# YuejiangDong/MAL

Measured on AMD Instinct MI355X. Metric: train images/sec at B=12 192x640 KITTI-shaped (MAL loss path: passes A+B+C fwd+bwd), higher is better.
Workload: dtype f32

## Files before the change

### mal_amd/csrc/mal_dyn.hip

```cpp
#include "mal_common.h"
#include "mal_device.h"

namespace mal {

MAL_DEV size_t dyn_row(const long long* sel, int i, int rows) {
  long long r = sel ? sel[i] : (long long)i;
  if (rows > 0) r = r < 0 ? 0 : (r >= rows ? (long long)rows - 1 : r);
  return (size_t)r;
}

struct DynParams {
  const uint8_t* mask_last; const uint8_t* mask_next;
  const long long* idx_last; const long long* idx_next;
  int rows_last, rows_next;
  int num, C, H, W, replace;
  const float* img_last; const float* img_next;
  float* ori_last; float* ori_next;
  int* ext;
  int* delta;
  uint8_t* flags;
  const float* g_ori_last; const float* g_ori_next; float* g_img_last; float* g_img_next;
  int prefilled;
  float* g_tmp_last; float* g_tmp_next;
};

constexpr int kDynBatch = 16;
struct DynBatch { DynParams s[kDynBatch]; };
constexpr int kExtChunks = 8;

__global__ __launch_bounds__(1024) void dyn_extents_kernel(DynBatch bt) {
  extern __shared__ int sh[];
  const DynParams& p = bt.s[blockIdx.z];
  if ((int)blockIdx.x >= p.num) return;
  const int i = blockIdx.x, which = blockIdx.y / kExtChunks, chunk = blockIdx.y % kExtChunks, tid = threadIdx.x;
  const int H = p.H, W = p.W;
  const int band = (H + kExtChunks - 1) / kExtChunks, r_lo = chunk * band, r_hi = min(r_lo + band, H);
  const int k_lo = r_lo * W, HW = max(r_hi, r_lo) * W;
  int* rowf = sh;
  int* colf = sh + H;
  int* res = sh + H + W;
  for (int k = tid; k < H + W; k += 1024) sh[k] = 0;
  if (tid < 4) res[tid] = (tid & 1) ? 0x7fffffff : 0;
  __syncthreads();
  const long long* sel = which ? p.idx_next : p.idx_last;
  const uint8_t* m = (which ? p.mask_next : p.mask_last) + dyn_row(sel, i, which ? p.rows_next : p.rows_last) * ((size_t)H * W);
  auto mark = [&](int k) { rowf[k / W] = 1; colf[k % W] = 1; };
  if ((HW & 15) == 0 && (k_lo & 15) == 0 && (reinterpret_cast<size_t>(m) & 15) == 0) {
    const uint4* m16 = reinterpret_cast<const uint4*>(m);
    for (int k = k_lo / 16 + tid; k < HW / 16; k += 1024) {
      const uint4 v = m16[k];
      const unsigned w4[4] = {v.x, v.y, v.z, v.w};
#pragma unroll
      for (int j = 0; j < 4; ++j)
        if (w4[j])
          for (int t = 0; t < 4; ++t)
            if ((w4[j] >> (8 * t)) & 0xffu) mark(k * 16 + j * 4 + t);
    }
  } else {
    for (int k = k_lo + tid; k < HW; k += 1024)
      if (m[k]) mark(k);
  }
  __syncthreads();
  for (int r = 1 + tid; r < H; r += 1024)
    if (rowf[r]) { atomicMax(&res[0], r); atomicMin(&res[1], r); }
  for (int c = 1 + tid; c < W; c += 1024)
    if (colf[c]) { atomicMax(&res[2], c); atomicMin(&res[3], c); }
  __syncthreads();
  if (tid < 4) p.ext[((i * 2 + which) * kExtChunks + chunk) * 4 + tid] = res[tid];
}

MAL_DEV unsigned nz4(unsigned w) {
  return ((w & 0xffu) ? 1u : 0u) | ((w & 0xff00u) ? 2u : 0u) | ((w & 0xff0000u) ? 4u : 0u) | ((w & 0xff000000u) ? 8u : 0u);
}

__global__ __launch_bounds__(1024) void dyn_extents16_kernel(DynBatch bt) {
  __shared__ int res[4];
  const DynParams& p = bt.s[blockIdx.z];
  if ((int)blockIdx.x >= p.num) return;
  const int i = blockIdx.x, which = blockIdx.y / kExtChunks, chunk = blockIdx.y % kExtChunks, tid = threadIdx.x;
  const int H = p.H, W = p.W, W16 = W >> 4;
  const int band = (H + kExtChunks - 1) / kExtChunks, r_lo = chunk * band, r_hi = min(r_lo + band, H);
  if (tid < 4) res[tid] = (tid & 1) ? 0x7fffffff : 0;
  __syncthreads();
  const long long* sel = which ? p.idx_next : p.idx_last;
  const uint4* m16 = reinterpret_cast<const uint4*>((which ? p.mask_next : p.mask_last) +
                                                    dyn_row(sel, i, which ? p.rows_next : p.rows_last) * ((size_t)H * W));
  int rmax = 0, rmin = 0x7fffffff, cmax = 0, cmin = 0x7fffffff;
  for (int k = r_lo * W16 + tid; k < max(r_hi, r_lo) * W16; k += (int)blockDim.x) {
    const uint4 v = m16[k];
    const unsigned w4[4] = {v.x, v.y, v.z, v.w};
    unsigned m = 0u;
#pragma unroll
    for (int j = 0; j < 4; ++j) m |= nz4(w4[j]) << (4 * j);
    if (m) {
      const int row = k / W16, col0 = (k - row * W16) * 16;
      if (row >= 1) { rmax = max(rmax, row); rmin = min(rmin, row); }
      const unsigned m1 = col0 == 0 ? (m & ~1u) : m;
      if (m1) { cmax = max(cmax, col0 + 31 - __clz((int)m1)); cmin = min(cmin, col0 + __ffs((int)m1) - 1); }
    }
  }
  for (int o = 32; o > 0; o >>= 1) {
    rmax = max(rmax, __shfl_down(rmax, o, 64)); rmin = min(rmin, __shfl_down(rmin, o, 64));
    cmax = max(cmax, __shfl_down(cmax, o, 64)); cmin = min(cmin, __shfl_down(cmin, o, 64));
  }
  if ((tid & 63) == 0) {
    if (rmax > 0) { atomicMax(&res[0], rmax); atomicMin(&res[1], rmin); }
    if (cmax > 0) { atomicMax(&res[2], cmax); atomicMin(&res[3], cmin); }
  }
  __syncthreads();
  if (tid < 4) p.ext[((i * 2 + which) * kExtChunks + chunk) * 4 + tid] = res[tid];
}

MAL_DEV void instance_delta(const DynParams& p, int i, int* dx_out, int* dy_out) {
  int el[4], en[4];
#pragma unroll 1
  for (int which = 0; which < 2; ++which) {
    int* e = which ? en : el;
    for (int t = 0; t < 4; ++t) e[t] = (t & 1) ? 0x7fffffff : 0;
    for (int c = 0; c < kExtChunks; ++c)
      for (int t = 0; t < 4; ++t) {
        const int v = p.ext[((i * 2 + which) * kExtChunks + c) * 4 + t];
        e[t] = (t & 1) ? min(e[t], v) : max(e[t], v);
      }
    for (int t = 0; t < 4; ++t)
      if (e[t] == 0x7fffffff) e[t] = 0;
  }
  auto pick = [](int a, int b) {
    const int s = abs(b) > abs(a) ? b : a;
    return (int)rintf((float)s * 0.5f);
  };
  int dx = pick(en[0] - el[0], en[1] - el[1]);
  int dy = pick(en[2] - el[2], en[3] - el[3]);
  if (p.replace) { if (abs(dx) < 3) dx = 0; if (abs(dy) < 3) dy = 0; }
  *dx_out = dx; *dy_out = dy;
}

MAL_DEV void stage_instances(const DynParams& p, int* s_delta, bool from_ext) {
  if (from_ext) {
    for (int i = threadIdx.x; i < p.num; i += 256) {
      int dx, dy;
      instance_delta(p, i, &dx, &dy);
      s_delta[2 * i] = dx; s_delta[2 * i + 1] = dy;
      if (blockIdx.x == 0) { p.delta[2 * i] = dx; p.delta[2 * i + 1] = dy; }
    }
  }
  for (int k = threadIdx.x; k < p.num * 2; k += 256) {
    if (!from_ext) s_delta[k] = p.delta[k];
    const int i = k >> 1;
    const long long* sel = (k & 1) ? p.idx_next : p.idx_last;
    s_delta[2 * p.num + k] = (int)dyn_row(sel, i, (k & 1) ? p.rows_next : p.rows_last);
  }
  __syncthreads();
}

__global__ __launch_bounds__(256) void dyn_synth_fwd_kernel(DynBatch bt) {
  extern __shared__ int s_delta[];
  const DynParams& p = bt.s[blockIdx.z];
  stage_instances(p, s_delta, true);
  const int* s_row = s_delta + 2 * p.num;
  const int H = p.H, W = p.W, HW = H * W;
  const int pix = blockIdx.x * 256 + threadIdx.x;
  if (pix >= HW) return;
  const int r = pix / W, c = pix - r * W;
  bool region = false, any_l = false, any_n = false, bg_l = false, bg_n = false;
  float accl[4] = {0.f, 0.f, 0.f, 0.f}, accn[4] = {0.f, 0.f, 0.f, 0.f};
  for (int i = 0; i < p.num; ++i) {
    const uint8_t* ml = p.mask_last + (size_t)s_row[2 * i] * HW;
    const uint8_t* mn = p.mask_next + (size_t)s_row[2 * i + 1] * HW;
    const bool a = ml[pix] != 0, b = mn[pix] != 0;
    region |= a | b; bg_l |= a & !b; bg_n |= b & !a;
    const int dx = s_delta[2 * i], dy = s_delta[2 * i + 1];
    {
      const int rs = r - dx, cs = c - dy;
      if (rs >= 0 && rs < H && cs >= 0 && cs < W && ml[rs * W + cs]) {
        any_l = true;
        for (int ch = 0; ch < p.C; ++ch) accl[ch] += p.img_last[(size_t)ch * HW + rs * W + cs];
      }
    }
    {
      const int rs = r + dx, cs = c + dy;
      if (rs >= 0 && rs < H && cs >= 0 && cs < W && mn[rs * W + cs]) {
        any_n = true;
        for (int ch = 0; ch < p.C; ++ch) accn[ch] += p.img_next[(size_t)ch * HW + rs * W + cs];
      }
    }
  }
  p.flags[pix] = (uint8_t)((region ? 1 : 0) | (any_l ? 2 : 0) | (any_n ? 4 : 0) | (bg_l ? 8 : 0) | (bg_n ? 16 : 0));
  if (p.prefilled && !region) return;
  for (int ch = 0; ch < p.C; ++ch) {
    const float il = p.img_last[(size_t)ch * HW + pix], in = p.img_next[(size_t)ch * HW + pix];
    p.ori_last[(size_t)ch * HW + pix] = region ? (any_l ? accl[ch] : (bg_l ? in : il)) : il;
    p.ori_next[(size_t)ch * HW + pix] = region ? (any_n ? accn[ch] : (bg_n ? il : in)) : in;
  }
}

template <bool REGION>
__global__ __launch_bounds__(256) void dyn_synth_bwd_kernel(DynBatch bt) {
  extern __shared__ int s_delta[];
  const DynParams& p = bt.s[blockIdx.z];
  stage_instances(p, s_delta, false);
  const int* s_row = s_delta + 2 * p.num;
  const int H = p.H, W = p.W, HW = H * W;
  const int pix = blockIdx.x * 256 + threadIdx.x;
  if (pix >= HW) return;
  const int r = pix / W, c = pix - r * W;
  const int f = p.flags[pix];
  if (REGION && !(f & 1)) return;
  const bool ol_from_l = !(f & 1) || (!(f & 2) && !(f & 8)), ol_from_n = (f & 1) && !(f & 2) && (f & 8);
  const bool on_from_n = !(f & 1) || (!(f & 4) && !(f & 16)), on_from_l = (f & 1) && !(f & 4) && (f & 16);
  float gl[4] = {0.f, 0.f, 0.f, 0.f}, gn[4] = {0.f, 0.f, 0.f, 0.f};
  for (int ch = 0; ch < p.C; ++ch) {
    const float a = p.g_ori_last[(size_t)ch * HW + pix], b = p.g_ori_next[(size_t)ch * HW + pix];
    if (ol_from_l) gl[ch] += a;
    if (on_from_l) gl[ch] += b;
    if (on_from_n) gn[ch] += b;
    if (ol_from_n) gn[ch] += a;
  }
  for (int i = 0; i < p.num; ++i) {
    const int dx = s_delta[2 * i], dy = s_delta[2 * i + 1];
    if (p.mask_last[(size_t)s_row[2 * i] * HW + pix]) {
      const int rd = r + dx, cd = c + dy;
      if (rd >= 0 && rd < H && cd >= 0 && cd < W && (p.flags[rd * W + cd] & 1))
        for (int ch = 0; ch < p.C; ++ch) gl[ch] += p.g_ori_last[(size_t)ch * HW + rd * W + cd];
    }
    if (p.mask_next[(size_t)s_row[2 * i + 1] * HW + pix]) {
      const int rd = r - dx, cd = c - dy;
      if (rd >= 0 && rd < H && cd >= 0 && cd < W && (p.flags[rd * W + cd] & 1))
        for (int ch = 0; ch < p.C; ++ch) gn[ch] += p.g_ori_next[(size_t)ch * HW + rd * W + cd];
    }
  }
  float* const out_l = REGION ? p.g_tmp_last : p.g_img_last;
  float* const out_n = REGION ? p.g_tmp_next : p.g_img_next;
  for (int ch = 0; ch < p.C; ++ch) {
    if (out_l) out_l[(size_t)ch * HW + pix] = gl[ch];
    if (out_n) out_n[(size_t)ch * HW + pix] = gn[ch];
  }
}

__global__ __launch_bounds__(256) void dyn_apply_region_kernel(DynBatch bt) {
  const DynParams& p = bt.s[blockIdx.z];
  const int HW = p.H * p.W;
  const int pix = blockIdx.x * 256 + threadIdx.x;
  if (pix >= HW || !(p.flags[pix] & 1)) return;
  for (int ch = 0; ch < p.C; ++ch) {
    p.g_img_last[(size_t)ch * HW + pix] = p.g_tmp_last[(size_t)ch * HW + pix];
    p.g_img_next[(size_t)ch * HW + pix] = p.g_tmp_next[(size_t)ch * HW + pix];
  }
}

MAL_DEV unsigned bytes4_at(const uint8_t* row, int cs, int W) {
  const unsigned* rw = reinterpret_cast<const unsigned*>(row);
  const int a0 = cs >> 2, sh = (cs & 3) * 8, wmax = (W >> 2) - 1;
  const unsigned l0 = rw[min(max(a0, 0), wmax)], l1 = rw[min(max(a0 + 1, 0), wmax)];
  const unsigned w0 = (a0 >= 0 && a0 <= wmax) ? l0 : 0u, w1 = (a0 + 1 >= 0 && a0 + 1 <= wmax) ? l1 : 0u;
  return sh ? (w0 >> sh) | (w1 << (32 - sh)) : w0;
}

MAL_DEV float4 ld4(const float* p) { return *reinterpret_cast<const float4*>(p); }
MAL_DEV void st4(float* p, const float (&v)[4]) { *reinterpret_cast<float4*>(p) = make_float4(v[0], v[1], v[2], v[3]); }

template <int C>
MAL_DEV void gather_add(float (&acc)[4][C], const float* __restrict__ img, int HW, unsigned sel, int base) {
  const char* plane[C];
#pragma unroll
  for (int ch = 0; ch < C; ++ch) {
    plane[ch] = reinterpret_cast<const char*>(img + (size_t)ch * HW);
    asm volatile("" : "+s"(plane[ch]));
  }
  float v[4][C];
#pragma unroll
  for (int k = 0; k < 4; ++k) {
    const unsigned off = (unsigned)(((sel >> k) & 1u) ? base + k : 0) * 4u;
#pragma unroll
    for (int ch = 0; ch < C; ++ch) v[k][ch] = *(const __attribute__((address_space(1))) float*)(plane[ch] + off);
  }
#pragma unroll
  for (int k = 0; k < 4; ++k)
#pragma unroll
    for (int ch = 0; ch < C; ++ch) {
      acc[k][ch] += ((sel >> k) & 1u) ? v[k][ch] : 0.f;
      asm volatile("" : "+v"(acc[k][ch]));
    }
}

template <int C>
__global__ __launch_bounds__(256) void dyn_synth_fwd4_kernel(DynBatch bt) {
  extern __shared__ int s_delta[];
  const DynParams& p = bt.s[blockIdx.z];
  stage_instances(p, s_delta, true);
  const int* s_row = s_delta + 2 * p.num;
  const int H = p.H, W = p.W, HW = H * W, W4 = W >> 2;
  const int q = blockIdx.x * 256 + threadIdx.x;
  if (q >= (HW >> 2)) return;
  const int r = q / W4, c = (q - r * W4) * 4, pix = r * W + c;
  const float* __restrict__ il = p.img_last;
  const float* __restrict__ in = p.img_next;
  unsigned region = 0u, any_l = 0u, any_n = 0u, bg_l = 0u, bg_n = 0u;
  float accl[4][C], accn[4][C];
#pragma unroll
  for (int k = 0; k < 4; ++k)
#pragma unroll
    for (int ch = 0; ch < C; ++ch) { accl[k][ch] = 0.f; accn[k][ch] = 0.f; }
  for (int i = 0; i < p.num; ++i) {
    const uint8_t* ml = p.mask_last + (size_t)__builtin_amdgcn_readfirstlane(s_row[2 * i]) * HW;
    const uint8_t* mn = p.mask_next + (size_t)__builtin_amdgcn_readfirstlane(s_row[2 * i + 1]) * HW;
    const int dx = __builtin_amdgcn_readfirstlane(s_delta[2 * i]), dy = __builtin_amdgcn_readfirstlane(s_delta[2 * i + 1]);
    const int rl = r - dx, rn = r + dx;
    const unsigned wa = *reinterpret_cast<const unsigned*>(ml + pix), wb = *reinterpret_cast<const unsigned*>(mn + pix);
    const unsigned sl_raw = bytes4_at(ml + (size_t)min(max(rl, 0), H - 1) * W, c - dy, W);
    const unsigned sn_raw = bytes4_at(mn + (size_t)min(max(rn, 0), H - 1) * W, c + dy, W);
    const unsigned a4 = nz4(wa), b4 = nz4(wb);
    const unsigned sl = (rl >= 0 && rl < H) ? nz4(sl_raw) : 0u, sn = (rn >= 0 && rn < H) ? nz4(sn_raw) : 0u;
    region |= a4 | b4; bg_l |= a4 & ~b4; bg_n |= b4 & ~a4;
    any_l |= sl; any_n |= sn;
    if (__any((sl | sn) != 0u)) {
      const int bl = rl * W + (c - dy), bn = rn * W + (c + dy);
      gather_add<C>(accl, il, HW, sl, bl);
      __builtin_amdgcn_sched_barrier(0);
      gather_add<C>(accn, in, HW, sn, bn);
    }
  }
  unsigned fw = 0u;
#pragma unroll
  for (int k = 0; k < 4; ++k)
    fw |= ((((region >> k) & 1u)) | (((any_l >> k) & 1u) << 1) | (((any_n >> k) & 1u) << 2) | (((bg_l >> k) & 1u) << 3) |
           (((bg_n >> k) & 1u) << 4)) << (8 * k);
  *reinterpret_cast<unsigned*>(p.flags + pix) = fw;
  if (p.prefilled && !__any(region != 0u)) return;
  const bool prefilled = p.prefilled != 0;
#pragma unroll
  for (int ch = 0; ch < C; ++ch) {
    const float4 a = ld4(il + (size_t)ch * HW + pix), b = ld4(in + (size_t)ch * HW + pix);
    const float av[4] = {a.x, a.y, a.z, a.w}, bv[4] = {b.x, b.y, b.z, b.w};
    float ol[4], on[4];
#pragma unroll
    for (int k = 0; k < 4; ++k) {
      const bool rg = (region >> k) & 1u;
      ol[k] = rg ? (((any_l >> k) & 1u) ? accl[k][ch] : (((bg_l >> k) & 1u) ? bv[k] : av[k])) : av[k];
      on[k] = rg ? (((any_n >> k) & 1u) ? accn[k][ch] : (((bg_n >> k) & 1u) ? av[k] : bv[k])) : bv[k];
    }
    float* const dl = p.ori_last + (size_t)ch * HW + pix;
    float* const dn = p.ori_next + (size_t)ch * HW + pix;
    if (!prefilled) { st4(dl, ol); st4(dn, on); continue; }
#pragma unroll
    for (int k = 0; k < 4; ++k)
      if ((region >> k) & 1u) { dl[k] = ol[k]; dn[k] = on[k]; }
  }
}

template <int C, bool REGION>
__global__ __launch_bounds__(256) void dyn_synth_bwd4_kernel(DynBatch bt) {
  extern __shared__ int s_delta[];
  const DynParams& p = bt.s[blockIdx.z];
  stage_instances(p, s_delta, false);
  const int* s_row = s_delta + 2 * p.num;
  const int H = p.H, W = p.W, HW = H * W, W4 = W >> 2;
  const int q = blockIdx.x * 256 + threadIdx.x;
  if (q >= (HW >> 2)) return;
  const int r = q / W4, c = (q - r * W4) * 4, pix = r * W + c;
  const float* __restrict__ go_l = p.g_ori_last;
  const float* __restrict__ go_n = p.g_ori_next;
  const unsigned fw = *reinterpret_cast<const unsigned*>(p.flags + pix);
  float* const out_l = REGION ? p.g_tmp_last : p.g_img_last;
  float* const out_n = REGION ? p.g_tmp_next : p.g_img_next;
  const bool wave_region = __any((fw & 0x01010101u) != 0u);
  if (REGION && !wave_region) return;
  float gl[C][4], gn[C][4];
#pragma unroll
  for (int ch = 0; ch < C; ++ch) {
    const float4 a4 = ld4(go_l + (size_t)ch * HW + pix), b4 = ld4(go_n + (size_t)ch * HW + pix);
    const float a[4] = {a4.x, a4.y, a4.z, a4.w}, b[4] = {b4.x, b4.y, b4.z, b4.w};
#pragma unroll
    for (int k = 0; k < 4; ++k) {
      const int f = (int)((fw >> (8 * k)) & 0xffu);
      const bool ol_from_l = !(f & 1) || (!(f & 2) && !(f & 8)), ol_from_n = (f & 1) && !(f & 2) && (f & 8);
      const bool on_from_n = !(f & 1) || (!(f & 4) && !(f & 16)), on_from_l = (f & 1) && !(f & 4) && (f & 16);
      float l = 0.f, n = 0.f;
      l += ol_from_l ? a[k] : 0.f;
      l += on_from_l ? b[k] : 0.f;
      n += on_from_n ? b[k] : 0.f;
      n += ol_from_n ? a[k] : 0.f;
      gl[ch][k] = l; gn[ch][k] = n;
    }
  }
  if (wave_region) {
    for (int i = 0; i < p.num; ++i) {
      const int dx = s_delta[2 * i], dy = s_delta[2 * i + 1];
      const unsigned ma = nz4(*reinterpret_cast<const unsigned*>(p.mask_last + (size_t)s_row[2 * i] * HW + pix));
      const unsigned mb = nz4(*reinterpret_cast<const unsigned*>(p.mask_next + (size_t)s_row[2 * i + 1] * HW + pix));
      const int rdl = r + dx, rdn = r - dx;
      const unsigned fl = bytes4_at(p.flags + (size_t)min(max(rdl, 0), H - 1) * W, c + dy, W);
      const unsigned fn = bytes4_at(p.flags + (size_t)min(max(rdn, 0), H - 1) * W, c - dy, W);
      unsigned hl = 0u, hn = 0u;
#pragma unroll
      for (int k = 0; k < 4; ++k) {
        hl |= (((fl >> (8 * k)) & 1u) & ((ma >> k) & 1u)) << k;
        hn |= (((fn >> (8 * k)) & 1u) & ((mb >> k) & 1u)) << k;
      }
      if (rdl < 0 || rdl >= H) hl = 0u;
      if (rdn < 0 || rdn >= H) hn = 0u;
      if (__any((hl | hn) != 0u)) {
        const int bl = rdl * W + (c + dy), bn = rdn * W + (c - dy);
        float vl[C][4], vn[C][4];
#pragma unroll
        for (int ch = 0; ch < C; ++ch)
#pragma unroll
          for (int k = 0; k < 4; ++k) {
            vl[ch][k] = go_l[(size_t)ch * HW + (((hl >> k) & 1u) ? bl + k : 0)];
            vn[ch][k] = go_n[(size_t)ch * HW + (((hn >> k) & 1u) ? bn + k : 0)];
          }
#pragma unroll
        for (int ch = 0; ch < C; ++ch)
#pragma unroll
          for (int k = 0; k < 4; ++k) {
            gl[ch][k] += ((hl >> k) & 1u) ? vl[ch][k] : 0.f;
            gn[ch][k] += ((hn >> k) & 1u) ? vn[ch][k] : 0.f;
          }
      }
    }
  }
  if (!REGION) {
#pragma unroll
    for (int ch = 0; ch < C; ++ch) {
      if (out_l) st4(out_l + (size_t)ch * HW + pix, gl[ch]);
      if (out_n) st4(out_n + (size_t)ch * HW + pix, gn[ch]);
    }
    return;
  }
#pragma unroll
  for (int k = 0; k < 4; ++k)
    if ((fw >> (8 * k)) & 1u) {
#pragma unroll
      for (int ch = 0; ch < C; ++ch) { out_l[(size_t)ch * HW + pix + k] = gl[ch][k]; out_n[(size_t)ch * HW + pix + k] = gn[ch][k]; }
    }
}

template <int C>
__global__ __launch_bounds__(256) void dyn_apply_region4_kernel(DynBatch bt) {
  const DynParams& p = bt.s[blockIdx.z];
  const int HW = p.H * p.W;
  const int q = blockIdx.x * 256 + threadIdx.x;
  if (q >= (HW >> 2)) return;
  const int pix = q * 4;
  const unsigned fw = *reinterpret_cast<const unsigned*>(p.flags + pix);
  if (!__any((fw & 0x01010101u) != 0u)) return;
  const float* __restrict__ tl = p.g_tmp_last;
  const float* __restrict__ tn = p.g_tmp_next;
  float4 vl[C], vn[C];
#pragma unroll
  for (int ch = 0; ch < C; ++ch) { vl[ch] = ld4(tl + (size_t)ch * HW + pix); vn[ch] = ld4(tn + (size_t)ch * HW + pix); }
#pragma unroll
  for (int ch = 0; ch < C; ++ch) {
    const float a[4] = {vl[ch].x, vl[ch].y, vl[ch].z, vl[ch].w}, b[4] = {vn[ch].x, vn[ch].y, vn[ch].z, vn[ch].w};
#pragma unroll
    for (int k = 0; k < 4; ++k)
      if ((fw >> (8 * k)) & 1u) { p.g_img_last[(size_t)ch * HW + pix + k] = a[k]; p.g_img_next[(size_t)ch * HW + pix + k] = b[k]; }
  }
}

}
namespace mal { opt_t g_dyn_small_blocks{1}; }

using namespace mal;

static bool aligned_to(const void* ptr, size_t a) { return ptr == nullptr || (reinterpret_cast<uintptr_t>(ptr) & (a - 1)) == 0; }

static int dyn_check(int num, int C, int H, int W) {
  if (num < 1 || num > MAL_MAX_INSTANCES || C < 1 || C > 4) return MAL_EINVAL;
  if (H < 2 || W < 2 || (double)H * W > 2.0e9 / 4) return MAL_ESHAPE;
  return MAL_OK;
}

extern "C" size_t mal_dyn_workspace_bytes(int num) {
  return num > 0 ? align256((size_t)num * 8 * kExtChunks * sizeof(int)) : 0;
}

static int dyn_fwd_chunk(const mal_dyn_item* it, int n, int C, int H, int W, int replace, hipStream_t st) {
  DynBatch bt = {};
  int max_num = 0;
  for (int k = 0; k < n; ++k) {
    const mal_dyn_item& a = it[k];
    int rc = dyn_check(a.num, C, H, W);
    if (rc) return rc;
    if (!a.mask_last || !a.mask_next || !a.img_last || !a.img_next || !a.ori_last || !a.ori_next || !a.delta || !a.flags ||
        !a.ws)
      return MAL_EINVAL;
    if (a.ws_bytes < mal_dyn_workspace_bytes(a.num)) return MAL_EWORKSPACE;
    DynParams& p = bt.s[k];
    p.mask_last = a.mask_last; p.mask_next = a.mask_next; p.num = a.num; p.C = C; p.H = H; p.W = W; p.replace = replace;
    p.idx_last = (const long long*)a.idx_last; p.idx_next = (const long long*)a.idx_next;
    p.rows_last = a.n_last; p.rows_next = a.n_next;
    p.img_last = a.img_last; p.img_next = a.img_next; p.ori_last = a.ori_last; p.ori_next = a.ori_next;
    p.ext = (int*)a.ws; p.delta = a.delta; p.flags = a.flags; p.prefilled = a.prefilled;
    max_num = a.num > max_num ? a.num : max_num;
  }
  bool wide = (W & 15) == 0;
  for (int k = 0; k < n && wide; ++k) wide = aligned_to(bt.s[k].mask_last, 16) && aligned_to(bt.s[k].mask_next, 16);
  if (wide)
    hipLaunchKernelGGL(dyn_extents16_kernel, dim3(max_num, 2 * kExtChunks, n), dim3(g_dyn_small_blocks ? 256 : 1024), 0, st, bt);
  else
    hipLaunchKernelGGL(dyn_extents_kernel, dim3(max_num, 2 * kExtChunks, n), dim3(1024), (size_t)(H + W + 4) * sizeof(int), st, bt);
  bool quad = (W & 3) == 0 && C == 3;
  for (int k = 0; k < n && quad; ++k) {
    const DynParams& q = bt.s[k];
    quad = aligned_to(q.mask_last, 4) && aligned_to(q.mask_next, 4) && aligned_to(q.flags, 4) && aligned_to(q.img_last, 16) &&
           aligned_to(q.img_next, 16) && aligned_to(q.ori_last, 16) && aligned_to(q.ori_next, 16);
  }
  if (quad)
    hipLaunchKernelGGL(dyn_synth_fwd4_kernel<3>, dim3((H * W / 4 + 255) / 256, 1, n), dim3(256), (size_t)max_num * 4 * sizeof(int), st, bt);
  else
    hipLaunchKernelGGL(dyn_synth_fwd_kernel, dim3((H * W + 255) / 256, 1, n), dim3(256), (size_t)max_num * 4 * sizeof(int), st, bt);
  return launch_status();
}

static int dyn_bwd_chunk(const mal_dyn_item* it, int n, int C, int H, int W, hipStream_t st) {
  DynBatch bt = {};
  int max_num = 0;
  int region = 0;
  for (int k = 0; k < n; ++k) {
    const mal_dyn_item& a = it[k];
    int rc = dyn_check(a.num, C, H, W);
    if (rc) return rc;
    if (!a.mask_last || !a.mask_next || !a.delta || !a.flags || !a.g_ori_last || !a.g_ori_next ||
        (!a.g_img_last && !a.g_img_next))
      return MAL_EINVAL;
    DynParams& p = bt.s[k];
    p.mask_last = a.mask_last; p.mask_next = a.mask_next; p.num = a.num; p.C = C; p.H = H; p.W = W;
    p.idx_last = (const long long*)a.idx_last; p.idx_next = (const long long*)a.idx_next;
    p.rows_last = a.n_last; p.rows_next = a.n_next;
    p.delta = a.delta; p.flags = a.flags;
    p.g_ori_last = a.g_ori_last; p.g_ori_next = a.g_ori_next; p.g_img_last = a.g_img_last; p.g_img_next = a.g_img_next;
    p.g_tmp_last = a.g_tmp_last; p.g_tmp_next = a.g_tmp_next;
    const bool inplace = a.g_img_last == a.g_ori_last || a.g_img_next == a.g_ori_next;
    if (inplace && (a.g_img_last != a.g_ori_last || a.g_img_next != a.g_ori_next || !a.g_tmp_last || !a.g_tmp_next)) return MAL_EINVAL;
    if (a.region_only) {
      if (inplace || !a.g_img_last || !a.g_img_next) return MAL_EINVAL;
      p.g_tmp_last = a.g_img_last; p.g_tmp_next = a.g_img_next;
    }
    const int form = a.region_only ? 2 : (inplace ? 1 : 0);
    if (k == 0) region = form;
    else if (region != form) return MAL_EINVAL;
    max_num = a.num > max_num ? a.num : max_num;
  }
  bool quad = (W & 3) == 0 && C == 3;
  for (int k = 0; k < n && quad; ++k) {
    const DynParams& q = bt.s[k];
    quad = aligned_to(q.mask_last, 4) && aligned_to(q.mask_next, 4) && aligned_to(q.flags, 4) && aligned_to(q.g_ori_last, 16) && aligned_to(q.g_ori_next, 16) && aligned_to(q.g_img_last, 16) &&
           aligned_to(q.g_img_next, 16) && aligned_to(q.g_tmp_last, 16) && aligned_to(q.g_tmp_next, 16);
  }
  const size_t lds = (size_t)max_num * 4 * sizeof(int);
  const dim3 grid((H * W + 255) / 256, 1, n), grid4((H * W / 4 + 255) / 256, 1, n);
  if (region && quad) {
    hipLaunchKernelGGL((dyn_synth_bwd4_kernel<3, true>), grid4, dim3(256), lds, st, bt);
    if (region == 1) hipLaunchKernelGGL(dyn_apply_region4_kernel<3>, grid4, dim3(256), 0, st, bt);
  } else if (region) {
    hipLaunchKernelGGL(dyn_synth_bwd_kernel<true>, grid, dim3(256), lds, st, bt);
    if (region == 1) hipLaunchKernelGGL(dyn_apply_region_kernel, grid, dim3(256), 0, st, bt);
  } else if (quad) {
    hipLaunchKernelGGL((dyn_synth_bwd4_kernel<3, false>), grid4, dim3(256), lds, st, bt);
  } else {
    hipLaunchKernelGGL(dyn_synth_bwd_kernel<false>, grid, dim3(256), lds, st, bt);
  }
  return launch_status();
}

extern "C" int mal_dyn_batch_fwd(const mal_dyn_item* items, int n_items, int C, int H, int W, int replace, void* stream) {
  if (!items || n_items < 1) return MAL_EINVAL;
  for (int o = 0; o < n_items; o += kDynBatch) {
    int rc = dyn_fwd_chunk(items + o, n_items - o < kDynBatch ? n_items - o : kDynBatch, C, H, W, replace, (hipStream_t)stream);
    if (rc) return rc;
  }
  return MAL_OK;
}

extern "C" int mal_dyn_batch_bwd(const mal_dyn_item* items, int n_items, int C, int H, int W, void* stream) {
  if (!items || n_items < 1) return MAL_EINVAL;
  for (int o = 0; o < n_items; o += kDynBatch) {
    int rc = dyn_bwd_chunk(items + o, n_items - o < kDynBatch ? n_items - o : kDynBatch, C, H, W, (hipStream_t)stream);
    if (rc) return rc;
  }
  return MAL_OK;
}

extern "C" int mal_dyn_instance_fwd(const uint8_t* mask_last, const uint8_t* mask_next, int num, const float* img_last,
                                    const float* img_next, int C, int H, int W, int replace, float* ori_last,
                                    float* ori_next, int32_t* delta, uint8_t* flags, void* ws, size_t ws_bytes,
                                    void* stream) {
  mal_dyn_item a = {};
  a.mask_last = mask_last; a.mask_next = mask_next; a.num = num; a.img_last = img_last; a.img_next = img_next;
  a.ori_last = ori_last; a.ori_next = ori_next; a.delta = delta; a.flags = flags; a.ws = ws; a.ws_bytes = ws_bytes;
  return dyn_fwd_chunk(&a, 1, C, H, W, replace, (hipStream_t)stream);
}

extern "C" int mal_dyn_instance_bwd(const uint8_t* mask_last, const uint8_t* mask_next, int num, const int32_t* delta,
                                    const uint8_t* flags, const float* g_ori_last, const float* g_ori_next, int C, int H,
                                    int W, float* g_img_last, float* g_img_next, void* stream) {
  mal_dyn_item a = {};
  a.mask_last = mask_last; a.mask_next = mask_next; a.num = num; a.delta = const_cast<int32_t*>(delta);
  a.flags = const_cast<uint8_t*>(flags); a.g_ori_last = g_ori_last; a.g_ori_next = g_ori_next;
  a.g_img_last = g_img_last; a.g_img_next = g_img_next;
  return dyn_bwd_chunk(&a, 1, C, H, W, (hipStream_t)stream);
}
```

Measured before the change: 42480.

## Batch instance mask loads in groups and prefetch cotangents in dynamic synth kernels

The forward and backward 4-pixel synth kernels now process instances in groups of three. All mask and flag word loads for a group are issued together before any use, and the backward kernel prefetches the next group and issues cotangent loads before shared-memory staging. Instance staging is reorganised so one thread per (instance, frame) reduces the extents and exchanges them via a shuffle, using a packed int4 record per instance. The extents scan also unrolls four uint4 loads per iteration. These changes aim to hide global-load latency and cut serial per-instance overhead, at the cost of more registers and a forced waves-per-EU setting that could limit occupancy or cause spills.

```diff
diff --git a/mal_amd/csrc/mal_dyn.hip b/mal_amd/csrc/mal_dyn.hip
--- a/mal_amd/csrc/mal_dyn.hip
+++ b/mal_amd/csrc/mal_dyn.hip
@@ -23,6 +23,15 @@
   int prefilled;
   float* g_tmp_last; float* g_tmp_next;
 };
+
+MAL_DEV int dyn_row_of_frame(const DynParams& p, int i, int which) {
+  long long rl = i, rn = i;
+  if (p.idx_last) rl = p.idx_last[i];
+  if (p.idx_next) rn = p.idx_next[i];
+  if (p.rows_last > 0) rl = rl < 0 ? 0 : (rl >= p.rows_last ? (long long)p.rows_last - 1 : rl);
+  if (p.rows_next > 0) rn = rn < 0 ? 0 : (rn >= p.rows_next ? (long long)p.rows_next - 1 : rn);
+  return (int)(which ? rn : rl);
+}
 
 constexpr int kDynBatch = 16;
 struct DynBatch { DynParams s[kDynBatch]; };
@@ -86,8 +95,7 @@
   const uint4* m16 = reinterpret_cast<const uint4*>((which ? p.mask_next : p.mask_last) +
                                                     dyn_row(sel, i, which ? p.rows_next : p.rows_last) * ((size_t)H * W));
   int rmax = 0, rmin = 0x7fffffff, cmax = 0, cmin = 0x7fffffff;
-  for (int k = r_lo * W16 + tid; k < max(r_hi, r_lo) * W16; k += (int)blockDim.x) {
-    const uint4 v = m16[k];
+  auto fold = [&](int k, const uint4& v) {
     const unsigned w4[4] = {v.x, v.y, v.z, v.w};
     unsigned m = 0u;
 #pragma unroll
@@ -98,6 +106,15 @@
       const unsigned m1 = col0 == 0 ? (m & ~1u) : m;
       if (m1) { cmax = max(cmax, col0 + 31 - __clz((int)m1)); cmin = min(cmin, col0 + __ffs((int)m1) - 1); }
     }
+  };
+  const int k_end = max(r_hi, r_lo) * W16, step = (int)blockDim.x;
+  for (int k = r_lo * W16 + tid; k < k_end; k += 4 * step) {
+    int kk[4];
+    uint4 v[4];
+#pragma unroll
+    for (int j = 0; j < 4; ++j) { kk[j] = min(k + j * step, k_end - 1); v[j] = m16[kk[j]]; }
+#pragma unroll
+    for (int j = 0; j < 4; ++j) fold(kk[j], v[j]);
   }
   for (int o = 32; o > 0; o >>= 1) {
     rmax = max(rmax, __shfl_down(rmax, o, 64)); rmin = min(rmin, __shfl_down(rmin, o, 64));
@@ -111,44 +128,49 @@
   if (tid < 4) p.ext[((i * 2 + which) * kExtChunks + chunk) * 4 + tid] = res[tid];
 }
 
-MAL_DEV void instance_delta(const DynParams& p, int i, int* dx_out, int* dy_out) {
-  int el[4], en[4];
-#pragma unroll 1
-  for (int which = 0; which < 2; ++which) {
-    int* e = which ? en : el;
-    for (int t = 0; t < 4; ++t) e[t] = (t & 1) ? 0x7fffffff : 0;
+static_assert(2 * MAL_MAX_INSTANCES <= 256, "stage_extents: one thread per (instance, frame) of a 256-thread workgroup");
+MAL_DEV void stage_extents(const DynParams& p, int* s_delta) {
+  const int t = threadIdx.x;
+  if (t < 2 * p.num) {
+    const int i = t >> 1, which = t & 1;
+    const int* rec = p.ext + (size_t)t * (kExtChunks * 4);
+    int v[kExtChunks][4];
+#pragma unroll
     for (int c = 0; c < kExtChunks; ++c)
-      for (int t = 0; t < 4; ++t) {
-        const int v = p.ext[((i * 2 + which) * kExtChunks + c) * 4 + t];
-        e[t] = (t & 1) ? min(e[t], v) : max(e[t], v);
-      }
-    for (int t = 0; t < 4; ++t)
-      if (e[t] == 0x7fffffff) e[t] = 0;
-  }
-  auto pick = [](int a, int b) {
-    const int s = abs(b) > abs(a) ? b : a;
-    return (int)rintf((float)s * 0.5f);
-  };
-  int dx = pick(en[0] - el[0], en[1] - el[1]);
-  int dy = pick(en[2] - el[2], en[3] - el[3]);
-  if (p.replace) { if (abs(dx) < 3) dx = 0; if (abs(dy) < 3) dy = 0; }
-  *dx_out = dx; *dy_out = dy;
-}
-
-MAL_DEV void stage_instances(const DynParams& p, int* s_delta, bool from_ext) {
-  if (from_ext) {
-    for (int i = threadIdx.x; i < p.num; i += 256) {
-      int dx, dy;
-      instance_delta(p, i, &dx, &dy);
-      s_delta[2 * i] = dx; s_delta[2 * i + 1] = dy;
+#pragma unroll
+      for (int k = 0; k < 4; ++k) v[c][k] = rec[c * 4 + k];
+    const int row = dyn_row_of_frame(p, i, which);
+    int e[4], o[4];
+#pragma unroll
+    for (int k = 0; k < 4; ++k) {
+      e[k] = (k & 1) ? 0x7fffffff : 0;
+#pragma unroll
+      for (int c = 0; c < kExtChunks; ++c) e[k] = (k & 1) ? min(e[k], v[c][k]) : max(e[k], v[c][k]);
+      if (e[k] == 0x7fffffff) e[k] = 0;
+      o[k] = __shfl_xor(e[k], 1, 64);
+    }
+    s_delta[4 * i + 2 + which] = row;
+    if (!which) {
+      auto pick = [](int a, int b) {
+        const int s = abs(b) > abs(a) ? b : a;
+        return (int)rintf((float)s * 0.5f);
+      };
+      int dx = pick(o[0] - e[0], o[1] - e[1]);
+      int dy = pick(o[2] - e[2], o[3] - e[3]);
+      if (p.replace) { if (abs(dx) < 3) dx = 0; if (abs(dy) < 3) dy = 0; }
+      s_delta[4 * i] = dx; s_delta[4 * i + 1] = dy;
       if (blockIdx.x == 0) { p.delta[2 * i] = dx; p.delta[2 * i + 1] = dy; }
     }
   }
-  for (int k = threadIdx.x; k < p.num * 2; k += 256) {
-    if (!from_ext) s_delta[k] = p.delta[k];
-    const int i = k >> 1;
-    const long long* sel = (k & 1) ? p.idx_next : p.idx_last;
-    s_delta[2 * p.num + k] = (int)dyn_row(sel, i, (k & 1) ? p.rows_next : p.rows_last);
+  __syncthreads();
+}
+
+MAL_DEV void stage_instances(const DynParams& p, int* s_delta) {
+  const int k = threadIdx.x;
+  if (k < 2 * p.num) {
+    const int i = k >> 1, d = p.delta[k], row = dyn_row_of_frame(p, i, k & 1);
+    s_delta[4 * i + (k & 1)] = d;
+    s_delta[4 * i + 2 + (k & 1)] = row;
   }
   __syncthreads();
 }
@@ -156,8 +178,7 @@
 __global__ __launch_bounds__(256) void dyn_synth_fwd_kernel(DynBatch bt) {
   extern __shared__ int s_delta[];
   const DynParams& p = bt.s[blockIdx.z];
-  stage_instances(p, s_delta, true);
-  const int* s_row = s_delta + 2 * p.num;
+  stage_extents(p, s_delta);
   const int H = p.H, W = p.W, HW = H * W;
   const int pix = blockIdx.x * 256 + threadIdx.x;
   if (pix >= HW) return;
@@ -165,11 +186,11 @@
   bool region = false, any_l = false, any_n = false, bg_l = false, bg_n = false;
   float accl[4] = {0.f, 0.f, 0.f, 0.f}, accn[4] = {0.f, 0.f, 0.f, 0.f};
   for (int i = 0; i < p.num; ++i) {
-    const uint8_t* ml = p.mask_last + (size_t)s_row[2 * i] * HW;
-    const uint8_t* mn = p.mask_next + (size_t)s_row[2 * i + 1] * HW;
+    const uint8_t* ml = p.mask_last + (size_t)s_delta[4 * i + 2] * HW;
+    const uint8_t* mn = p.mask_next + (size_t)s_delta[4 * i + 3] * HW;
     const bool a = ml[pix] != 0, b = mn[pix] != 0;
     region |= a | b; bg_l |= a & !b; bg_n |= b & !a;
-    const int dx = s_delta[2 * i], dy = s_delta[2 * i + 1];
+    const int dx = s_delta[4 * i], dy = s_delta[4 * i + 1];
     {
       const int rs = r - dx, cs = c - dy;
       if (rs >= 0 && rs < H && cs >= 0 && cs < W && ml[rs * W + cs]) {
@@ -198,8 +219,7 @@
 __global__ __launch_bounds__(256) void dyn_synth_bwd_kernel(DynBatch bt) {
   extern __shared__ int s_delta[];
   const DynParams& p = bt.s[blockIdx.z];
-  stage_instances(p, s_delta, false);
-  const int* s_row = s_delta + 2 * p.num;
+  stage_instances(p, s_delta);
   const int H = p.H, W = p.W, HW = H * W;
   const int pix = blockIdx.x * 256 + threadIdx.x;
   if (pix >= HW) return;
@@ -217,13 +237,13 @@
     if (ol_from_n) gn[ch] += a;
   }
   for (int i = 0; i < p.num; ++i) {
-    const int dx = s_delta[2 * i], dy = s_delta[2 * i + 1];
-    if (p.mask_last[(size_t)s_row[2 * i] * HW + pix]) {
+    const int dx = s_delta[4 * i], dy = s_delta[4 * i + 1];
+    if (p.mask_last[(size_t)s_delta[4 * i + 2] * HW + pix]) {
       const int rd = r + dx, cd = c + dy;
       if (rd >= 0 && rd < H && cd >= 0 && cd < W && (p.flags[rd * W + cd] & 1))
         for (int ch = 0; ch < p.C; ++ch) gl[ch] += p.g_ori_last[(size_t)ch * HW + rd * W + cd];
     }
-    if (p.mask_next[(size_t)s_row[2 * i + 1] * HW + pix]) {
+    if (p.mask_next[(size_t)s_delta[4 * i + 3] * HW + pix]) {
       const int rd = r - dx, cd = c - dy;
       if (rd >= 0 && rd < H && cd >= 0 && cd < W && (p.flags[rd * W + cd] & 1))
         for (int ch = 0; ch < p.C; ++ch) gn[ch] += p.g_ori_next[(size_t)ch * HW + rd * W + cd];
@@ -248,78 +268,123 @@
   }
 }
 
-MAL_DEV unsigned bytes4_at(const uint8_t* row, int cs, int W) {
-  const unsigned* rw = reinterpret_cast<const unsigned*>(row);
+
+MAL_DEV unsigned ldw(const uint8_t* base, unsigned off) {
+  const char* b = reinterpret_cast<const char*>(base);
+  asm volatile("" : "+s"(b));
+  return *(const __attribute__((address_space(1))) unsigned*)(b + off);
+}
+MAL_DEV void bytes4_ld(const uint8_t* plane, int row, int cs, int W, unsigned (&l)[2]) {
+  const int a0 = cs >> 2, wmax = (W >> 2) - 1;
+  const unsigned o = (unsigned)(row * W);
+  l[0] = ldw(plane, o + 4u * (unsigned)min(max(a0, 0), wmax)); l[1] = ldw(plane, o + 4u * (unsigned)min(max(a0 + 1, 0), wmax));
+}
+MAL_DEV unsigned bytes4_mix(const unsigned (&l)[2], int cs, int W) {
   const int a0 = cs >> 2, sh = (cs & 3) * 8, wmax = (W >> 2) - 1;
-  const unsigned l0 = rw[min(max(a0, 0), wmax)], l1 = rw[min(max(a0 + 1, 0), wmax)];
-  const unsigned w0 = (a0 >= 0 && a0 <= wmax) ? l0 : 0u, w1 = (a0 + 1 >= 0 && a0 + 1 <= wmax) ? l1 : 0u;
+  const unsigned w0 = (a0 >= 0 && a0 <= wmax) ? l[0] : 0u, w1 = (a0 + 1 >= 0 && a0 + 1 <= wmax) ? l[1] : 0u;
   return sh ? (w0 >> sh) | (w1 << (32 - sh)) : w0;
 }
+MAL_DEV void arrived(unsigned& v) { asm volatile("" : "+v"(v)); }
 
 MAL_DEV float4 ld4(const float* p) { return *reinterpret_cast<const float4*>(p); }
 MAL_DEV void st4(float* p, const float (&v)[4]) { *reinterpret_cast<float4*>(p) = make_float4(v[0], v[1], v[2], v[3]); }
 
 template <int C>
-MAL_DEV void gather_add(float (&acc)[4][C], const float* __restrict__ img, int HW, unsigned sel, int base) {
+MAL_DEV void gather_ld(float (&v)[4][C], const float* __restrict__ img, int HW, unsigned sel, int base) {
   const char* plane[C];
 #pragma unroll
   for (int ch = 0; ch < C; ++ch) {
     plane[ch] = reinterpret_cast<const char*>(img + (size_t)ch * HW);
     asm volatile("" : "+s"(plane[ch]));
   }
-  float v[4][C];
 #pragma unroll
   for (int k = 0; k < 4; ++k) {
     const unsigned off = (unsigned)(((sel >> k) & 1u) ? base + k : 0) * 4u;
 #pragma unroll
     for (int ch = 0; ch < C; ++ch) v[k][ch] = *(const __attribute__((address_space(1))) float*)(plane[ch] + off);
   }
+}
+template <int C, bool PIN>
+MAL_DEV void gather_acc(float (&acc)[4][C], const float (&v)[4][C], unsigned sel) {
 #pragma unroll
   for (int k = 0; k < 4; ++k)
 #pragma unroll
     for (int ch = 0; ch < C; ++ch) {
       acc[k][ch] += ((sel >> k) & 1u) ? v[k][ch] : 0.f;
-      asm volatile("" : "+v"(acc[k][ch]));
-    }
-}
-
+      if (PIN) asm volatile("" : "+v"(acc[k][ch]));
+    }
+}
 template <int C>
-__global__ __launch_bounds__(256) void dyn_synth_fwd4_kernel(DynBatch bt) {
+MAL_DEV void gather_add(float (&acc)[4][C], const float* __restrict__ img, int HW, unsigned sel, int base) {
+  float v[4][C];
+  gather_ld<C>(v, img, HW, sel, base);
+  gather_acc<C, true>(acc, v, sel);
+}
+
+constexpr int kSynthGroup = 3;
+static_assert(kSynthGroup >= 1 && kSynthGroup <= 4, "dyn_synth_fwd4_kernel: a byte of `hits` per instance of the group");
+
+template <int C>
+__global__ __launch_bounds__(256) __attribute__((amdgpu_waves_per_eu(8, 8))) void dyn_synth_fwd4_kernel(DynBatch bt) {
   extern __shared__ int s_delta[];
   const DynParams& p = bt.s[blockIdx.z];
-  stage_instances(p, s_delta, true);
-  const int* s_row = s_delta + 2 * p.num;
+  stage_extents(p, s_delta);
   const int H = p.H, W = p.W, HW = H * W, W4 = W >> 2;
   const int q = blockIdx.x * 256 + threadIdx.x;
   if (q >= (HW >> 2)) return;
   const int r = q / W4, c = (q - r * W4) * 4, pix = r * W + c;
   const float* __restrict__ il = p.img_last;
   const float* __restrict__ in = p.img_next;
-  unsigned region = 0u, any_l = 0u, any_n = 0u, bg_l = 0u, bg_n = 0u;
+  unsigned pred = 0u;
   float accl[4][C], accn[4][C];
 #pragma unroll
   for (int k = 0; k < 4; ++k)
 #pragma unroll
     for (int ch = 0; ch < C; ++ch) { accl[k][ch] = 0.f; accn[k][ch] = 0.f; }
-  for (int i = 0; i < p.num; ++i) {
-    const uint8_t* ml = p.mask_last + (size_t)__builtin_amdgcn_readfirstlane(s_row[2 * i]) * HW;
-    const uint8_t* mn = p.mask_next + (size_t)__builtin_amdgcn_readfirstlane(s_row[2 * i + 1]) * HW;
-    const int dx = __builtin_amdgcn_readfirstlane(s_delta[2 * i]), dy = __builtin_amdgcn_readfirstlane(s_delta[2 * i + 1]);
-    const int rl = r - dx, rn = r + dx;
-    const unsigned wa = *reinterpret_cast<const unsigned*>(ml + pix), wb = *reinterpret_cast<const unsigned*>(mn + pix);
-    const unsigned sl_raw = bytes4_at(ml + (size_t)min(max(rl, 0), H - 1) * W, c - dy, W);
-    const unsigned sn_raw = bytes4_at(mn + (size_t)min(max(rn, 0), H - 1) * W, c + dy, W);
-    const unsigned a4 = nz4(wa), b4 = nz4(wb);
-    const unsigned sl = (rl >= 0 && rl < H) ? nz4(sl_raw) : 0u, sn = (rn >= 0 && rn < H) ? nz4(sn_raw) : 0u;
-    region |= a4 | b4; bg_l |= a4 & ~b4; bg_n |= b4 & ~a4;
-    any_l |= sl; any_n |= sn;
-    if (__any((sl | sn) != 0u)) {
-      const int bl = rl * W + (c - dy), bn = rn * W + (c + dy);
+  for (int i0 = 0; i0 < p.num; i0 += kSynthGroup) {
+    unsigned hits = 0u;
+    unsigned wa[kSynthGroup], wb[kSynthGroup], wl[kSynthGroup][2], wn[kSynthGroup][2];
+    int dxs[kSynthGroup], dys[kSynthGroup];
+#pragma unroll
+    for (int j = 0; j < kSynthGroup; ++j) {
+      const int4 rec = *reinterpret_cast<const int4*>(s_delta + 4 * min(i0 + j, p.num - 1));
+      const int dx = dxs[j] = __builtin_amdgcn_readfirstlane(rec.x), dy = dys[j] = __builtin_amdgcn_readfirstlane(rec.y);
+      const uint8_t* ml = p.mask_last + (size_t)__builtin_amdgcn_readfirstlane(rec.z) * HW;
+      const uint8_t* mn = p.mask_next + (size_t)__builtin_amdgcn_readfirstlane(rec.w) * HW;
+      wa[j] = ldw(ml, (unsigned)pix); wb[j] = ldw(mn, (unsigned)pix);
+      bytes4_ld(ml, min(max(r - dx, 0), H - 1), c - dy, W, wl[j]);
+      bytes4_ld(mn, min(max(r + dx, 0), H - 1), c + dy, W, wn[j]);
+    }
+    __builtin_amdgcn_sched_barrier(0);
+#pragma unroll
+    for (int j = 0; j < kSynthGroup; ++j) {
+      arrived(wa[j]); arrived(wb[j]); arrived(wl[j][0]); arrived(wl[j][1]); arrived(wn[j][0]); arrived(wn[j][1]);
+    }
+#pragma unroll
+    for (int j = 0; j < kSynthGroup; ++j) {
+      const bool live = i0 + j < p.num;
+      const int rl = r - dxs[j], rn = r + dxs[j];
+      const unsigned a4 = live ? nz4(wa[j]) : 0u, b4 = live ? nz4(wb[j]) : 0u;
+      const unsigned sl = (live && rl >= 0 && rl < H) ? nz4(bytes4_mix(wl[j], c - dys[j], W)) : 0u;
+      const unsigned sn = (live && rn >= 0 && rn < H) ? nz4(bytes4_mix(wn[j], c + dys[j], W)) : 0u;
+      pred |= (a4 | b4) | (sl << 4) | (sn << 8) | ((a4 & ~b4) << 12) | ((b4 & ~a4) << 16);
+      hits |= (sl | (sn << 4)) << (8 * j);
+    }
+    if (!__any(hits != 0u)) continue;
+#pragma unroll 1
+    for (int j = 0; j < kSynthGroup; ++j) {
+      const unsigned sl = (hits >> (8 * j)) & 15u, sn = (hits >> (8 * j + 4)) & 15u;
+      if (!__any((sl | sn) != 0u)) continue;
+      const int i = i0 + j;
+      const int dx = __builtin_amdgcn_readfirstlane(s_delta[4 * i]), dy = __builtin_amdgcn_readfirstlane(s_delta[4 * i + 1]);
+      const int bl = (r - dx) * W + (c - dy), bn = (r + dx) * W + (c + dy);
       gather_add<C>(accl, il, HW, sl, bl);
       __builtin_amdgcn_sched_barrier(0);
       gather_add<C>(accn, in, HW, sn, bn);
     }
   }
+  const unsigned region = pred & 15u, any_l = (pred >> 4) & 15u, any_n = (pred >> 8) & 15u, bg_l = (pred >> 12) & 15u,
+                 bg_n = (pred >> 16) & 15u;
   unsigned fw = 0u;
 #pragma unroll
   for (int k = 0; k < 4; ++k)
@@ -352,24 +417,45 @@
 __global__ __launch_bounds__(256) void dyn_synth_bwd4_kernel(DynBatch bt) {
   extern __shared__ int s_delta[];
   const DynParams& p = bt.s[blockIdx.z];
-  stage_instances(p, s_delta, false);
-  const int* s_row = s_delta + 2 * p.num;
   const int H = p.H, W = p.W, HW = H * W, W4 = W >> 2;
   const int q = blockIdx.x * 256 + threadIdx.x;
-  if (q >= (HW >> 2)) return;
-  const int r = q / W4, c = (q - r * W4) * 4, pix = r * W + c;
+  const bool inside = q < (HW >> 2);
+  const int qc = inside ? q : 0;
+  const int r = qc / W4, c = (qc - r * W4) * 4, pix = r * W + c;
   const float* __restrict__ go_l = p.g_ori_last;
   const float* __restrict__ go_n = p.g_ori_next;
+  float4 ct_l[C], ct_n[C];
+  auto request_cotangents = [&]() {
+#pragma unroll
+    for (int ch = 0; ch < C; ++ch) { ct_l[ch] = ld4(go_l + (size_t)ch * HW + pix); ct_n[ch] = ld4(go_n + (size_t)ch * HW + pix); }
+  };
   const unsigned fw = *reinterpret_cast<const unsigned*>(p.flags + pix);
+  if (!REGION) request_cotangents();
+  stage_instances(p, s_delta);
+  if (!inside) return;
   float* const out_l = REGION ? p.g_tmp_last : p.g_img_last;
   float* const out_n = REGION ? p.g_tmp_next : p.g_img_next;
   const bool wave_region = __any((fw & 0x01010101u) != 0u);
   if (REGION && !wave_region) return;
-  float gl[C][4], gn[C][4];
+  if (REGION) request_cotangents();
+  unsigned wm[kSynthGroup][2], wf[kSynthGroup][2][2];
+  int dxs[kSynthGroup], dys[kSynthGroup];
+  auto request_group = [&](int i0) {
+#pragma unroll
+    for (int j = 0; j < kSynthGroup; ++j) {
+      const int4 rec = *reinterpret_cast<const int4*>(s_delta + 4 * min(i0 + j, p.num - 1));
+      const int dx = dxs[j] = __builtin_amdgcn_readfirstlane(rec.x), dy = dys[j] = __builtin_amdgcn_readfirstlane(rec.y);
+      wm[j][0] = ldw(p.mask_last + (size_t)__builtin_amdgcn_readfirstlane(rec.z) * HW, (unsigned)pix);
+      wm[j][1] = ldw(p.mask_next + (size_t)__builtin_amdgcn_readfirstlane(rec.w) * HW, (unsigned)pix);
+      bytes4_ld(p.flags, min(max(r + dx, 0), H - 1), c + dy, W, wf[j][0]);
+      bytes4_ld(p.flags, min(max(r - dx, 0), H - 1), c - dy, W, wf[j][1]);
+    }
+  };
+  if (wave_region) request_group(0);
+  float gl[4][C], gn[4][C];
 #pragma unroll
   for (int ch = 0; ch < C; ++ch) {
-    const float4 a4 = ld4(go_l + (size_t)ch * HW + pix), b4 = ld4(go_n + (size_t)ch * HW + pix);
-    const float a[4] = {a4.x, a4.y, a4.z, a4.w}, b[4] = {b4.x, b4.y, b4.z, b4.w};
+    const float a[4] = {ct_l[ch].x, ct_l[ch].y, ct_l[ch].z, ct_l[ch].w}, b[4] = {ct_n[ch].x, ct_n[ch].y, ct_n[ch].z, ct_n[ch].w};
 #pragma unroll
     for (int k = 0; k < 4; ++k) {
       const int f = (int)((fw >> (8 * k)) & 0xffu);
@@ -380,50 +466,57 @@
       l += on_from_l ? b[k] : 0.f;
       n += on_from_n ? b[k] : 0.f;
       n += ol_from_n ? a[k] : 0.f;
-      gl[ch][k] = l; gn[ch][k] = n;
+      gl[k][ch] = l; gn[k][ch] = n;
     }
   }
   if (wave_region) {
-    for (int i = 0; i < p.num; ++i) {
-      const int dx = s_delta[2 * i], dy = s_delta[2 * i + 1];
-      const unsigned ma = nz4(*reinterpret_cast<const unsigned*>(p.mask_last + (size_t)s_row[2 * i] * HW + pix));
-      const unsigned mb = nz4(*reinterpret_cast<const unsigned*>(p.mask_next + (size_t)s_row[2 * i + 1] * HW + pix));
-      const int rdl = r + dx, rdn = r - dx;
-      const unsigned fl = bytes4_at(p.flags + (size_t)min(max(rdl, 0), H - 1) * W, c + dy, W);
-      const unsigned fn = bytes4_at(p.flags + (size_t)min(max(rdn, 0), H - 1) * W, c - dy, W);
-      unsigned hl = 0u, hn = 0u;
-#pragma unroll
-      for (int k = 0; k < 4; ++k) {
-        hl |= (((fl >> (8 * k)) & 1u) & ((ma >> k) & 1u)) << k;
-        hn |= (((fn >> (8 * k)) & 1u) & ((mb >> k) & 1u)) << k;
+    for (int i0 = 0;;) {
+      __builtin_amdgcn_sched_barrier(0);
+#pragma unroll
+      for (int j = 0; j < kSynthGroup; ++j) {
+        arrived(wm[j][0]); arrived(wm[j][1]); arrived(wf[j][0][0]); arrived(wf[j][0][1]); arrived(wf[j][1][0]); arrived(wf[j][1][1]);
       }
-      if (rdl < 0 || rdl >= H) hl = 0u;
-      if (rdn < 0 || rdn >= H) hn = 0u;
-      if (__any((hl | hn) != 0u)) {
-        const int bl = rdl * W + (c + dy), bn = rdn * W + (c - dy);
-        float vl[C][4], vn[C][4];
-#pragma unroll
-        for (int ch = 0; ch < C; ++ch)
-#pragma unroll
-          for (int k = 0; k < 4; ++k) {
-            vl[ch][k] = go_l[(size_t)ch * HW + (((hl >> k) & 1u) ? bl + k : 0)];
-            vn[ch][k] = go_n[(size_t)ch * HW + (((hn >> k) & 1u) ? bn + k : 0)];
-          }
-#pragma unroll
-        for (int ch = 0; ch < C; ++ch)
-#pragma unroll
-          for (int k = 0; k < 4; ++k) {
-            gl[ch][k] += ((hl >> k) & 1u) ? vl[ch][k] : 0.f;
-            gn[ch][k] += ((hn >> k) & 1u) ? vn[ch][k] : 0.f;
-          }
+      unsigned hl[kSynthGroup], hn[kSynthGroup], any = 0u;
+#pragma unroll
+      for (int j = 0; j < kSynthGroup; ++j) {
+        const unsigned ma = nz4(wm[j][0]), mb = nz4(wm[j][1]);
+        const unsigned fl = bytes4_mix(wf[j][0], c + dys[j], W), fn = bytes4_mix(wf[j][1], c - dys[j], W);
+        const int rdl = r + dxs[j], rdn = r - dxs[j];
+        hl[j] = 0u; hn[j] = 0u;
+#pragma unroll
+        for (int k = 0; k < 4; ++k) {
+          hl[j] |= (((fl >> (8 * k)) & 1u) & ((ma >> k) & 1u)) << k;
+          hn[j] |= (((fn >> (8 * k)) & 1u) & ((mb >> k) & 1u)) << k;
+        }
+        const bool live = i0 + j < p.num;
+        if (!live || rdl < 0 || rdl >= H) hl[j] = 0u;
+        if (!live || rdn < 0 || rdn >= H) hn[j] = 0u;
+        any |= hl[j] | hn[j];
       }
+      if (__any(any != 0u)) {
+        float vl[kSynthGroup][4][C], vn[kSynthGroup][4][C];
+#pragma unroll
+        for (int j = 0; j < kSynthGroup; ++j) {
+          gather_ld<C>(vl[j], go_l, HW, hl[j], (r + dxs[j]) * W + (c + dys[j]));
+          gather_ld<C>(vn[j], go_n, HW, hn[j], (r - dxs[j]) * W + (c - dys[j]));
+        }
+#pragma unroll
+        for (int j = 0; j < kSynthGroup; ++j) {
+          gather_acc<C, false>(gl, vl[j], hl[j]);
+          gather_acc<C, false>(gn, vn[j], hn[j]);
+        }
+      }
+      i0 += kSynthGroup;
+      if (i0 >= p.num) break;
+      request_group(i0);
     }
   }
   if (!REGION) {
 #pragma unroll
     for (int ch = 0; ch < C; ++ch) {
-      if (out_l) st4(out_l + (size_t)ch * HW + pix, gl[ch]);
-      if (out_n) st4(out_n + (size_t)ch * HW + pix, gn[ch]);
+      const float ol[4] = {gl[0][ch], gl[1][ch], gl[2][ch], gl[3][ch]}, on[4] = {gn[0][ch], gn[1][ch], gn[2][ch], gn[3][ch]};
+      if (out_l) st4(out_l + (size_t)ch * HW + pix, ol);
+      if (out_n) st4(out_n + (size_t)ch * HW + pix, on);
     }
     return;
   }
@@ -431,7 +524,7 @@
   for (int k = 0; k < 4; ++k)
     if ((fw >> (8 * k)) & 1u) {
 #pragma unroll
-      for (int ch = 0; ch < C; ++ch) { out_l[(size_t)ch * HW + pix + k] = gl[ch][k]; out_n[(size_t)ch * HW + pix + k] = gn[ch][k]; }
+      for (int ch = 0; ch < C; ++ch) { out_l[(size_t)ch * HW + pix + k] = gl[k][ch]; out_n[(size_t)ch * HW + pix + k] = gn[k][ch]; }
     }
 }
 
```

Result: no change. 42740 (median of 6 runs) (+0.6%).
